# ebu/libear

Measured on AMD Instinct MI355X. Metric: Msamples/s, higher is better.
Workload: dtype f32 io / f16x2-split MFMA, f32 accumulate

## Files before the change

include/earhip.h:

```cpp
#ifndef EARHIP_H
#define EARHIP_H

#include <stddef.h>
#include <stdint.h>

#ifdef __cplusplus
extern "C" {
#endif

#define EARHIP_VERSION 100

#define EARHIP_OK 0
#define EARHIP_INVALID_ARGUMENT 1
#define EARHIP_INTERNAL_ERROR 2
#define EARHIP_DEVICE_ERROR 3
#define EARHIP_NOT_IMPLEMENTED 4
#define EARHIP_UNKNOWN_LAYOUT 5
#define EARHIP_ADM_ERROR 6

int earhip_version(void);
const char *earhip_last_error(void);
int earhip_device_count(int *count);

typedef struct earhip_ctx earhip_ctx;
// ... 231 lines not shown
int earhip_render_process_frames_pcm(earhip_render *r, size_t nblocks, const void *frames,
                                     earhip_pcm_format fmt, int frame_channels, int first_channel,
                                     void *out_frames, const earhip_pcm_out *out);
int earhip_render_process_frames_pcm_device(earhip_render *r, size_t nblocks, const void *frames_dev,
                                            earhip_pcm_format fmt, int frame_channels,
                                            int first_channel, void *out_dev, size_t out_frame_bytes,
                                            size_t out_first_byte, const earhip_pcm_out *out);
int earhip_render_output_levels(earhip_render *r, float *peak, uint64_t *clipped, int reset);
int earhip_render_enable_timing(earhip_render *r, int enable);
int earhip_render_get_timing(earhip_render *r, double out[6]);
int earhip_render_gain_kernel(const earhip_render *r, int *kind);
int earhip_render_hinge_standby(earhip_render *r, int *standby);
int earhip_render_hinge_robust(earhip_render *r, int *robust);
int earhip_render_wide_form(earhip_render *r, int *wide);
int earhip_render_last_plan(const earhip_render *r, int out[4]);
int earhip_render_last_list_layout(const earhip_render *r, int *paired);
int earhip_render_last_tail_blocks(const earhip_render *r, int *blocks);
int earhip_render_last_host_chunks(const earhip_render *r, int *chunks);
int earhip_render_scratch_bytes(const earhip_render *r, size_t *bytes);

typedef struct earhip_comm earhip_comm;
int earhip_comm_unique_id(void *id128);
int earhip_comm_create(earhip_ctx *ctx, int rank, int world, const void *id128, earhip_comm **out);
int earhip_comm_destroy(earhip_comm *comm);
int earhip_comm_channel_range(int n_out, int rank, int world, int *padded_rows, int *lo, int *hi);
int earhip_render_exchange_device(earhip_comm *comm, int slot, const float *partial_dev,
                                  float *owned_dev, size_t rows_per_rank, size_t row_stride);
int earhip_comm_gather_device(earhip_comm *comm, int slot, const float *owned_dev, float *full_dev,
                              size_t rows_per_rank, size_t row_stride, int root);
int earhip_comm_wait(earhip_comm *comm, int slot);
// ... 39 lines not shown
```

libear_amd/capi.py:

```python
import ctypes as C
import os

import numpy as np

from .build import lib_path

f32p = C.POINTER(C.c_float)
i64p = C.POINTER(C.c_int64)
pp_f32 = C.POINTER(f32p)

OK, INVALID_ARGUMENT, INTERNAL_ERROR, DEVICE_ERROR, NOT_IMPLEMENTED, UNKNOWN_LAYOUT, ADM_ERROR = 0, 1, 2, 3, 4, 5, 6


class EarHipError(Exception):
    def __init__(self, code, msg):
        super().__init__(msg)
        self.code = code


class InvalidArgument(EarHipError, ValueError):
    """maps to ear::invalid_argument"""


class InternalError(EarHipError, RuntimeError):
# ... 829 lines not shown
    def last_host_chunks(self):
        v = C.c_int(0)
        check(load().earhip_render_last_host_chunks(self.h, C.byref(v)))
        return v.value

    def last_list_layout(self):
        v = C.c_int(0)
        check(load().earhip_render_last_list_layout(self.h, C.byref(v)))
        return None if v.value < 0 else bool(v.value)

    def last_plan(self):
        out = (C.c_int * 4)()
        check(load().earhip_render_last_plan(self.h, out))
        return {"kernel": out[0], "tile": out[1], "ntiles": out[2], "gsplit": out[3]}

    def attach_loudness(self, meter):
        check(load().earhip_render_attach_loudness(self.h, meter.h if meter is not None else None))
        self._meter = meter

    def close(self):
        if self.h:
            load().earhip_render_destroy(self.h)
            self.h = C.c_void_p()



def _f64(a):
    return np.ascontiguousarray(a, dtype=np.float64)


# ... 106 lines not shown
```

libear_amd/csrc/api_core.hip:

```cpp
#include <cctype>
#include <cerrno>
#include <cmath>
#include <cstdlib>
#include <string>
#include <memory>
#include <mutex>

#include "common.h"
#include "curves.h"
#include "gain_kernels.h"
#include "gain_mfma.h"
#include "gain_h2.h"
#include "gain_h2_t1.h"
#include "gain_p2.h"
#include "gain_hg.h"
#include "gain_f32g.h"

namespace earhip {

static_assert(kSplitTile == 256, "MixLaunch::tile() and tiles_aligned(256, ...) assume the 4-wave tile");

static thread_local std::string g_last_error;
void set_last_error(const std::string &msg) { g_last_error = msg; }

// ... 140 lines not shown
    const dim3 bgrid((pnt + tpw - 1) / tpw);
    PairRec *stage = nullptr;
    if (ctx->has(OPT_BUILD_2K) ? ctx->get(OPT_BUILD_2K) != 0 : ml.paired) {
      stage = reinterpret_cast<PairRec *>(desc) + piece_units((size_t)M, (size_t)pnt, (size_t)pl.slots);
      hipLaunchKernelGGL(k_piece_classify, dim3((pnt + 63) / 64, (M + kClassifyObjects - 1) / kClassifyObjects), dim3(64 * kClassifyObjects), 0,
                         ctx->stream, ps, M, pnt, ptile, t_call, t_call + nsamples, pl.paired, stage, obj_lv, level_cur,
                         ml.hinge ? gate : nullptr);
    }
#define EARHIP_BUILD_CASE(T_)                                                                                          \
  if (tpw == T_)                                                                                                       \
    hipLaunchKernelGGL(k_piece_build<T_>, bgrid, dim3(kBuildThreads), 0, ctx->stream, ps, M, pnt, ptile, t_call, \
                       t_call + nsamples, pl, obj_lv, level_cur, ml.hinge ? gate : nullptr, ctx->obj_level_cap, wide_cur, stage);
    EARHIP_BUILD_CASE(1) EARHIP_BUILD_CASE(2) EARHIP_BUILD_CASE(4) EARHIP_BUILD_CASE(8)
#undef EARHIP_BUILD_CASE
  }
  if (!fused_prep && !one_pass) {
    const dim3 ogrid((M + 15) / 16);
    QuietMark qm;
    if (probe.obj_level) {
      qm.obj_level = probe.obj_level, qm.cap = ctx->obj_level_cap, qm.level = level_cur;
      qm.wide = ml.split ? wide_cur : nullptr;
    }
    if (ml.ntiles >= 2048)
      hipLaunchKernelGGL(k_seg_prep<4>, dim3((ml.ntiles + 63) / 64, ogrid.x), dim3(256), 0, ctx->stream, ps, M,
                         ml.ntiles, ml.tile(), t_call, t_call + nsamples, desc, qm, slow_cur);
    else
      hipLaunchKernelGGL(k_seg_prep<2>, dim3((ml.ntiles + 31) / 32, ogrid.x), dim3(256), 0, ctx->stream, ps, M,
                         ml.ntiles, ml.tile(), t_call, t_call + nsamples, desc, qm, slow_cur);
  }
  SlotLists sl;
  sl.slots = reinterpret_cast<Slot *>(desc + (size_t)M * ml.ntiles);
// ... 1 lines not shown
  sl.ovf = sl.count + (size_t)4 * ml.ntiles;
  sl.M = M;
  if (slots)
    hipLaunchKernelGGL(k_slot_list, dim3(ml.ntiles), dim3(256), 0, ctx->stream, ps, M, ml.tile(),
                       t_call, t_call + nsamples, fused_prep ? nullptr : desc, sl);
  if (ev) EARHIP_HIP(hipEventRecord(ev[1], ctx->stream));
  GainMixParams P;
  P.mode_word = gate;
  P.record = gate ? record : nullptr;
  P.sl = sl;
  P.in = in_dev;
  P.in_stride = in_stride;
  P.out = out_dev;
  P.out_stride = out_stride;
  P.part_stride = part_stride;
  P.desc = desc;
  P.ps = ps;
  P.t_call = t_call;
  P.nsamples = nsamples;
  P.ntiles = ml.ntiles;
  P.M = M;
  P.ncols = cs.ncols();
  P.ngroups = ml.mfma ? cp.mgroups : cp.ngroups;
  P.wsplit = ml.wsplit;
  P.tiles_per_wg = ml.mfma ? ml.tpw : 1;
  P.vec_ok = (in_stride % 4 == 0 && out_stride % 4 == 0 && part_stride % 4 == 0 &&
              ((uintptr_t)in_dev & 15) == 0 && ((uintptr_t)out_dev & 15) == 0)
                 ? 1
                 : 0;
  const dim3 grid(ml.mfma ? (ml.ntiles + ml.tpw - 1) / ml.tpw : ml.ntiles, ml.gsplit,
                  ml.mfma ? cp.mnz : cp.nz);
// ... 111 lines not shown
#undef EARHIP_MIX_CASE
  if (!launched) fail_internal("no gain_mix instantiation for this column plan");
  if (ev) EARHIP_HIP(hipEventRecord(ev[3], ctx->stream));
  EARHIP_HIP(hipGetLastError());
}

void reserve_call_words(earhip_ctx *ctx, int M, size_t max_samples) {
  if (!ctx->level.p) ctx->level.alloc_zero(4, ctx->stream);
  const size_t ntiles = (max_samples + 255) / 256;
  const bool grow_obj = ctx->obj_level_cap < M, grow_tiles = ctx->tile_slow_cap < ntiles;
  if (grow_obj || grow_tiles) EARHIP_HIP(hipStreamSynchronize(ctx->stream));
  if (grow_obj) {
    ctx->obj_level_cap = M + M / 2 + 64;
    ctx->obj_level.alloc_zero(2 * (size_t)ctx->obj_level_cap, ctx->stream);
  }
  if (grow_tiles) {
    ctx->tile_slow_cap = std::max<size_t>(ntiles + ntiles / 4, 1024);
    ctx->tile_slow.alloc_zero(2 * ctx->tile_slow_cap, ctx->stream);
    ctx->tile_slow_idx = 0;
  }
}

size_t hinge_build_allow_lds(const hipDeviceProp_t &prop) {
  const size_t want = 128 * 1024, dflt = 64 * 1024;
  const size_t device_max = std::max((size_t)prop.sharedMemPerBlock, (size_t)prop.maxSharedMemoryPerMultiProcessor);
  size_t ask = std::min(want, device_max > 4096 ? device_max - 4096 : dflt);
  if (ask <= dflt) return dflt;
  bool ok = true;
#define EARHIP_HBUILD_ATTR(T_, NW_)                                                                       \
  ok = ok && hipFuncSetAttribute(reinterpret_cast<const void *>(&k_hinge_build<T_, NW_>),                 \
// ... 58 lines not shown
    run_device(t_call, n, ctx->dev_in.p, stride, ctx->dev_out.p, stride);
    EARHIP_HIP(hipMemcpyAsync(ctx->pin_out.p, ctx->dev_out.p, sizeof(float) * stride * n_out,
                              hipMemcpyDeviceToHost, ctx->stream));
    EARHIP_HIP(hipStreamSynchronize(ctx->stream));
    for (int c = 0; c < n_out; c++)
      std::memcpy(out[c] + r0, ctx->pin_out.p + c * stride, sizeof(float) * n);
  }
};

}

using namespace earhip;

static const char *const kOptNames[OPT_COUNT] = {
    "SPL", "MFMA", "XSCALE", "WAVES", "TPW", "NRT", "H2_TILE", "H2_WGS", "H2_RUNS", "P2_TILE", "P2_PAIRS", "P2_WGS", "HINGE", "HG_TILE", "HBUILD_TPW",
    "BUILD_TPW", "K2_WG", "K2_OWN_BLOCK", "RUN", "GSPLIT", "PROBE_RUNS", "BLOCK_GROUPS", "DEBUG_TIMING", "TAILCUT", "HOST_CHUNK_MB", "HOST_THREADS", "HG_ROBUST", "BUILD_2K", "HOST_BIND", "HOST_NT", "HOST_FIRST", "H2_PAIR"};

static int parse_option_value(const std::string &key, const char *text) {
  char *end = nullptr;
  errno = 0;
  const long v = std::strtol(text, &end, 10);
  while (end && *end && std::isspace((unsigned char)*end)) end++;
  if (end == text || (end && *end) || errno == ERANGE || v < -(1L << 30) || v > (1L << 30))
    fail_invalid("option '" + key + "': '" + std::string(text) + "' is not an integer");
  return (int)v;
}

void earhip_ctx::apply_options() {
  spl = 4, use_mfma = 3, x_scale_log2 = 14, x_scale_auto = true, max_waves = 4, tiles_per_wg = 4, tiles_per_wg_forced = false, nrt = 8;
  if (has(OPT_SPL) && (get(OPT_SPL) == 2 || get(OPT_SPL) == 4)) spl = get(OPT_SPL);
  if (has(OPT_MFMA)) use_mfma = get(OPT_MFMA);
// ... 474 lines not shown
```

libear_amd/csrc/api_render.hip:

```cpp
#include <cmath>
#include <cstdlib>
#include <atomic>
#include <chrono>
#include <condition_variable>
#include <memory>
#include <mutex>
#include <thread>
#include <vector>


#include "common.h"
#include "curves.h"
#include "host_gather.h"
#include "pcm_kernels.h"
#include "pcm_out_kernels.h"
#include "fft_kernels.h"
#include "render_kernels.h"

using namespace earhip;

namespace earhip {
std::vector<cf> make_twiddles(int L) {
  std::vector<cf> tw(L);
  const double pi = 3.14159265358979323846264338327950288;
// ... 221 lines not shown
    }
    (void)hipStreamDestroy(in);
    (void)hipStreamDestroy(out);
  }
};

struct earhip_render {
  earhip_ctx *ctx = nullptr;
  int M = 0, N = 0, B = 0, K = 1, D = 0, T = 0;
  int Bk = 0, Lk = 0;
  int NP = 1;
  std::unique_ptr<CurveSet> curves;
  int64_t t = 0;
  int last_plan[3] = {0, 0, 0};
  int last_paired = -1;
  size_t last_scratch_bytes = 0;
  long scratch_regrows = 0;
  DevBuf<unsigned> rec;
  bool last_gated = false;
  bool last_device_form = false;
  bool last_hg_robust = false;
  int last_kind = -1;
  int run_len = 11;
  bool run_len_set = false;

  DevBuf<SegDesc> desc;
  DevBuf<float> bus;
  int max_gsplit = 1;
  DevBuf<cf> H, tw;
  DevBuf<float> tail[2], dly[2], hist[2];
// ... 266 lines not shown
        P.accumulate = part > 0 ? 1 : 0;
        if (wave_k2) {
          hipLaunchKernelGGL(k_decorrelate_wave, dim3((grid.x + kDecorWaves - 1) / kDecorWaves, grid.y), dim3(64 * kDecorWaves),
                             0, ctx->stream, P);
          EARHIP_HIP(hipGetLastError());
        } else {
          launch_decor(Lk, P, grid, ctx->stream, true);
        }
      }
      if (evp) EARHIP_HIP(hipEventRecord(evp[5], ctx->stream));
      cur ^= 1;
      fresh = false;
    }
    if (timed) pending.push_back(pd);
    last_gated = ctx->last_gate_idx >= 0;
    last_device_form = ctx->last_wide_idx >= 0;
    last_hg_robust = last_gated && ctx->last_hinge_robust;
    if (ctx->lazy_allocs != lazy_before) scratch_regrows++;
    t += nsamples;
  }
};

extern "C" {

int earhip_render_create(earhip_ctx *ctx, const earhip_render_config *cfg, earhip_render **out) {
  return guarded([&] {
    require(ctx != nullptr && cfg != nullptr && out != nullptr, "NULL argument");
    require(cfg->n_objects >= 1 && cfg->n_out >= 1, "n_objects and n_out must be >= 1");
    require(cfg->n_buses == 1 || cfg->n_buses == 2, "n_buses must be 1 or 2");
    FftShape shape;
// ... 706 lines not shown

int earhip_render_last_host_chunks(const earhip_render *r, int *chunks) {
  return guarded([&] {
    require(r != nullptr && chunks != nullptr, "NULL argument");
    *chunks = r->last_host_chunks;
  });
}

int earhip_render_last_list_layout(const earhip_render *r, int *paired) {
  return guarded([&] {
    require(r != nullptr && paired != nullptr, "NULL argument");
    *paired = r->last_paired;
  });
}

int earhip_render_last_plan(const earhip_render *r, int out[4]) {
  return guarded([&] {
    require(r != nullptr && out != nullptr, "NULL argument");
    out[0] = r->last_kind;
    for (int i = 0; i < 3; i++) out[1 + i] = r->last_plan[i];
  });
}

}
```

libear_amd/csrc/common.h:

```cpp
#pragma once

#include <hip/hip_runtime.h>

#include <cstdint>
#include <cstdio>
#include <string>
#include <vector>

#include "../../include/earhip.h"

namespace earhip {

struct Error {
  int code;
  std::string msg;
};

void set_last_error(const std::string &msg);

template <typename F>
int guarded(F &&f) {
  try {
    f();
    return EARHIP_OK;
// ... 79 lines not shown
};

}

struct earhip_vbs;
namespace earhip {
void vbs_orphan(earhip_vbs *v);
}

namespace earhip {
enum Opt {
  OPT_SPL, OPT_MFMA, OPT_XSCALE, OPT_WAVES, OPT_TPW, OPT_NRT,
  OPT_H2_TILE, OPT_H2_WGS, OPT_H2_RUNS, OPT_P2_TILE, OPT_P2_PAIRS, OPT_P2_WGS, OPT_HINGE, OPT_HG_TILE, OPT_HBUILD_TPW, OPT_BUILD_TPW,
  OPT_K2_WG, OPT_K2_OWN_BLOCK, OPT_RUN, OPT_GSPLIT,
  OPT_PROBE_RUNS, OPT_BLOCK_GROUPS, OPT_DEBUG_TIMING, OPT_TAILCUT, OPT_HOST_CHUNK_MB, OPT_HOST_THREADS, OPT_HG_ROBUST, OPT_BUILD_2K,
  OPT_HOST_BIND, OPT_HOST_NT, OPT_HOST_FIRST, OPT_H2_PAIR, OPT_COUNT
};
struct OptVal {
  bool set = false;
  int v = 0;
};
}

struct earhip_ctx {
  earhip::OptVal opt[earhip::OPT_COUNT];
  bool has(earhip::Opt o) const { return opt[o].set; }
  int get(earhip::Opt o, int dflt = 0) const { return opt[o].set ? opt[o].v : dflt; }
  void apply_options();
  int device = 0;
  hipStream_t stream = nullptr;
  bool own_stream = false;
  bool strict = false;
  int spl = 4;
  int use_mfma = 3;
  int x_scale_log2 = 14;
  bool x_scale_auto = true;
  earhip::DevBuf<unsigned> level;
  int level_idx = 0;
  int last_gate_idx = -1;
  bool last_hinge_robust = false;
  int last_wide_idx = -1;
  earhip::DevBuf<unsigned> tile_slow;
  size_t tile_slow_cap = 0;
  int tile_slow_idx = 0;
  earhip::DevBuf<unsigned> obj_level;
  int obj_level_cap = 0;
  long lazy_allocs = 0;
  unsigned *record_slot = nullptr;
  int max_waves = 4;
  int tiles_per_wg = 4;
  bool tiles_per_wg_forced = false;
  int nrt = 8;
  int num_cus = 256;
  size_t hinge_build_lds = 64 * 1024;
  struct HostRange {
    const char *base;
    size_t bytes;
    bool owned;
  };
  std::vector<HostRange> host_ranges;
  std::vector<earhip_vbs *> pinned_adapters;
// ... 24 lines not shown
```

libear_amd/csrc/curves.h:

```cpp
#pragma once

#include <chrono>
#include <cmath>
#include <cstdio>
#include <cstdlib>

#include <algorithm>
#include <cstring>
#include <vector>

#include "common.h"
#include "gain_kernels.h"
#include "gain_p2.h"
#include "gain_hg.h"
#include "gain_f32g.h"

namespace earhip {

struct ColumnPlan {
  int nout = 24;
  int ngroups = 1;
  int nz = 1;
  int nct = 1;
  int mgroups = 1;
  int mnz = 1;
  int row = 24;
  static ColumnPlan make(int ncols) {
    ColumnPlan p;
    int groups = (ncols + 23) / 24;
    const int per = (ncols + groups - 1) / groups;
// ... 25 lines not shown
  if (threadIdx.x == 0) dst.off[m] = off, dst.cnt[m] = n, dst.hdr[m] = src.hdr[m];
  for (int i = threadIdx.x; i < n; i += 256) {
    dst.time[off + i] = src.time[off + i];
    dst.flat[off + i] = src.flat[off + i];
    dst.rec[off + i] = src.rec[off + i];
  }
  const size_t g0 = (size_t)off * row, gn = (size_t)n * row;
  const float4 *sg = reinterpret_cast<const float4 *>(src.gain + g0);
  float4 *dg = reinterpret_cast<float4 *>(dst.gain + g0);
  for (size_t i = threadIdx.x; i < gn / 4; i += 256) dg[i] = sg[i];
}

class CurveSet {
 public:
  CurveSet(int M, int ncols, int nbus = 1, bool force_ramp = false)
      : M_(M), ncols_(ncols), nbus_(nbus), force_ramp_(force_ramp), plan_(ColumnPlan::make(ncols)), obj_(M) {
    for (int m = 0; m < M; m++) {
      obj_[m].t.assign(1, 0);
      obj_[m].g.assign(plan_.row, 0.0f);
      obj_[m].flat.assign(1, 0);
      obj_[m].dirty = true;
      dirty_list_.push_back(m);
    }
    cmax_.assign(plan_.row, 0.0f);
    obj_cmax_.assign((size_t)M * plan_.row, 0.0f);
    cm_scratch_.assign(plan_.row, 0.0f);
    shrunk_cols_.assign(plan_.row, 0);
    dirty_list_.reserve(M);
    for (auto &p : phases_) p.items.reserve(M);
  }
  ~CurveSet() {
// ... 135 lines not shown
      h_cnt_.p[m] = n;
      h_hdr_.p[m] = ObjHdr{o.off, n, o.t[0], o.t[n - 1], 0};
      std::memcpy(h_time_.p + o.off, o.t.data(), (size_t)n * sizeof(int64_t));
      std::memcpy(h_flat_.p + o.off, o.flat.data(), (size_t)n);
      std::memcpy(h_gain_.p + (size_t)o.off * row, o.g.data(), (size_t)n * row * sizeof(float));
      for (int k = 0; k < n; k++) {
        PointRec &r = h_rec_.p[o.off + k];
        r.time = o.t[k];
        const int64_t len = k ? o.t[k] - o.t[k - 1] : 0;
        r.scale = len > 0 ? 1.0f / (float)len : 0.0f;
        r.flat = o.flat[k];
      }
      float *cm = obj_cmax_.data() + (size_t)m * row;
      if (o.has_stats) cmax_shrunk = retire(o.st, cm) || cmax_shrunk;
      o.st = stats_of(o, cm);
      admit(o.st, cm);
      o.has_stats = true;
    }
    if (cmax_shrunk) {
      for (size_t c = 0; c < row; c++) {
        if (!shrunk_cols_[c]) continue;
        shrunk_cols_[c] = 0;
        float v = 0.0f;
        for (int m = 0; m < M_; m++) {
          const float a = obj_cmax_[(size_t)m * row + c];
          v = a <= v ? v : a;
        }
        cmax_[c] = v;
      }
    }
// ... 64 lines not shown

  int aligned_tile(int64_t t_call) const {
    const int grids[2] = {512, 256};
    for (int gi = 0; gi < 2; gi++) {
      const int64_t G = grids[gi];
      const int si = 1 - gi;
      int off_grid_limit = M_ / 64;
      if (ramp_share() < 0.5) {
        const double deltas = deltas_per_pair(si ? 512 : 256);
        off_grid_limit = (int)(M_ * std::min(1.0 / 64, deltas / 200.0));
      }
      if (tiles_aligned((int)G, t_call)) return (int)G;
      if (grid_off_[gi] <= off_grid_limit && (((t_call - grid_phase_[gi]) % G) + G) % G == 0) return (int)G;
    }
    return 0;
  }

  double deltas_per_pair(int tile) const {
    const int gi = tile >= 512 ? 1 : 0;
    return tot_.tiles[gi] > 0 ? tot_.incid[gi] / tot_.tiles[gi] * moving_share() : 0.0;
  }
  double moving_share() const { return M_ > 0 ? (double)tot_.moving / M_ : 0.0; }
  double point_density_all() const { return point_density() * moving_share(); }
  double ramp_share() const { return tot_.span > 0 ? tot_.ramp / tot_.span : 0.0; }
  double point_density() const { return tot_.span > 0 ? tot_.npts / tot_.span : 0.0; }
  double pair_waste(int tile) const {
    const int gi = tile >= 512 ? 1 : 0;
    return (tot_.incid[gi] - tot_.touched[gi]) / std::max(1.0, tot_.tiles[gi] + tot_.incid[gi]);
  }
  double hinge_exact_share(size_t in_stride, size_t nsamples) const {
// ... 171 lines not shown
        uint64_t b = g;
        while (a) {
          const uint64_t r = b % a;
          b = a;
          a = r;
        }
        g = b;
      };
      for (int m = 0; m < M_ && g != 1; m++) {
        const ObjStats &s = obj_[m].st;
        fold(s.gcd);
        fold((uint64_t)(s.first >= t_ref_ ? s.first - t_ref_ : t_ref_ - s.first));
      }
      grid_ = g;
      grid_stale_ = false;
    }
    for (int gi = 0; gi < 2; gi++) {
      int64_t best = 0;
      int best_n = 0;
      for (const auto &kv : phases_[gi].items)
        if (kv.second > best_n) best_n = kv.second, best = kv.first;
      grid_phase_[gi] = best;
      grid_off_[gi] = M_ - best_n;
    }
    float gmax = 0.0f;
    for (float v : cmax_) gmax = v <= gmax ? gmax : v;
    gain_max_ = gmax;
  }

  int M_, ncols_, nbus_;
  bool force_ramp_;
  ColumnPlan plan_;
  std::vector<Obj> obj_;
  std::vector<int> dirty_list_;
  bool uploaded_once_ = false;
  size_t arena_used_ = 2, arena_cap_ = 0, abandoned_ = 0;
  struct Totals {
    double span = 0, ramp = 0, npts = 0, bad = 0, points = 0;
    long moving = 0;
    double incid[2] = {0, 0}, touched[2] = {0, 0}, tiles[2] = {0, 0};
    long sum_r15[2] = {0, 0}, sum_r7[2] = {0, 0};
  } tot_;
  struct PhaseCounts {
    std::vector<std::pair<int64_t, int>> items;
    void add(int64_t phase, int d) {
      for (size_t i = 0; i < items.size(); i++)
        if (items[i].first == phase) {
          items[i].second += d;
          if (items[i].second <= 0) items[i] = items.back(), items.pop_back();
// ... 149 lines not shown
```

libear_amd/csrc/gain_h2.h:

```cpp
#pragma once

#include <hip/hip_runtime.h>

#include <type_traits>

#include "gain_kernels.h"
#include "gain_mfma.h"

namespace earhip {

typedef uint32_t u32x4 __attribute__((ext_vector_type(4)));
typedef float f32x2 __attribute__((ext_vector_type(2)));

constexpr int kSplitTile = 256;
constexpr int kSplitChunk = 32;

typedef _Float16 f16x8 __attribute__((ext_vector_type(8)));
typedef _Float16 f16x2_t __attribute__((ext_vector_type(2)));

__device__ __forceinline__ uint32_t pack_f16(float a, float b) {
  const f32x2 v = {a, b};
  return __builtin_bit_cast(uint32_t, __builtin_convertvector(v, f16x2_t));
}
__device__ __forceinline__ float f16_lo(uint32_t u) { return (float)__builtin_bit_cast(f16x2_t, u)[0]; }
// ... 220 lines not shown
      const int ts0 = st.tile * (TS * NW);
      const char *bp = reinterpret_cast<const char *>(P.in + (live ? (size_t)chunk_base(st.c) * P.in_stride + ts0 : 0));
      const size_t rstride = live ? P.in_stride * sizeof(float) : 0;
      const unsigned xo = live ? xrow + 4u * (unsigned)min(xsl, nvec - 4 - ts0) : 0u;
#pragma unroll
      for (int q = 0; q < 8; q++)
        if (q >= q0 && q < q0 + n)
          x[q] = __builtin_nontemporal_load(reinterpret_cast<const f32x4 *>(bp + (size_t)q * rstride + xo));
    };
    auto load_x = [&](const Stage &st, bool live, f32x4 (&x)[8]) { load_x_part(st, live, x, 0, 8); };
    typedef const SegDesc __attribute__((address_space(4))) *ConstDesc;
    struct ChunkDesc {
      SegDesc d[NQ];
    };
    auto load_desc = [&](const Stage &st) {
      ConstDesc dp = (ConstDesc)(P.desc + (size_t)st.tile * P.M + chunk_base(st.c) + w * NQ);
      ChunkDesc D;
#pragma unroll
      for (int q = 0; q < NQ; q++) {
        D.d[q].row = dp[q].row;
        D.d[q].d0 = dp[q].d0;
        D.d[q].scale = dp[q].scale;
        D.d[q].info = dp[q].info;
      }
      return D;
    };
    struct ChunkCoef {
      float p0[NQ], scale[NQ];
    };
    auto load_gains = [&](const ChunkDesc &R, int cc, ChunkCoef &D, float (&S)[NQ], float (&E)[NQ]) {
      const int m0 = chunk_base(cc) + w * NQ;
#pragma unroll
      for (int q = 0; q < NQ; q++) {
        const SegDesc d = R.d[q];
        const bool valid = m0 + q >= m_lo + cc * CH && !(d.info & (kSegMulti | kSegQuiet));
        const unsigned rs = (unsigned)(valid ? d.row : zero_row);
        const unsigned re = (valid && (d.info & kSegRamp)) ? (unsigned)d.row + 1u : rs;
        D.p0[q] = d.scale != 0.0f ? (float)(d.d0 + (TS * NW) / 2) * d.scale : 0.0f;
        D.scale[q] = d.scale;
        const float *rps = gain + (size_t)rs * rowlen, *rpe = gain + (size_t)re * rowlen;
        S[q] = rps[bcol_e];
        E[q] = rpe[bcol_e];
      }
    };
    auto store_b = [&](const ChunkCoef &D, const float (&S)[NQ], const float (&E)[NQ], int buf, int part) {
      uint32_t h[NQ / 2], l[NQ / 2], hs[NQ / 2];
#pragma unroll
      for (int i = 0; i < NQ / 2; i++) {
        float v[2];
// ... 22 lines not shown
      }
    };

    f32x4 X0[8], X1[8];
    ChunkDesc L;
    Stage sa, sb, sc;
    sa.tile = tile_at(vb_c);
    sa.c = 0;
    sb = next_stage(sa);
    sc = next_stage(sb);
    int ka = 0;
    {
      float S[NQ], E[NQ];
      ChunkCoef D;
      L = load_desc(sa);
      load_gains(L, 0, D, S, E);
      load_x(sa, true, X0);
      load_x(sb, left > 1, X1);
      store_b(D, S, E, 0, 0);
      store_b(D, S, E, 0, 1);
      L = load_desc(sb);
    }
    auto chunk = [&](int buf, f32x4 (&xc)[8]) __attribute__((always_inline)) {
      __syncthreads();
      float S[NQ], E[NQ];
      ChunkCoef D;
      load_gains(L, sb.c, D, S, E);
      L = load_desc(sc);
      __builtin_amdgcn_sched_barrier(0);

      u32x4 ah[NRT], al[NRT];
#pragma unroll
      for (int qp = 0; qp < 4; qp++)
#pragma unroll
        for (int rp = 0; rp < NRT; rp += 2) {
          const f32x2 s0 = f32x2{xc[2 * qp][rp], xc[2 * qp][rp + 1]} * x_scale;
          const f32x2 s1 = f32x2{xc[2 * qp + 1][rp], xc[2 * qp + 1][rp + 1]} * x_scale;
          const uint32_t H0 = pack_f16(s0[0], s1[0]), H1 = pack_f16(s0[1], s1[1]);
          constexpr float LOW = WIDE ? kLowPieceScale : 1.0f;
          const f32x2 r0 = f32x2{sub_f16_lo(s0[0], H0), sub_f16_lo(s0[1], H1)} * LOW;
          const f32x2 r1 = f32x2{sub_f16_hi(s1[0], H0), sub_f16_hi(s1[1], H1)} * LOW;
          ah[rp][qp] = H0;
// ... 54 lines not shown
            __builtin_amdgcn_sched_group_barrier(0x002, 2, 0);
            __builtin_amdgcn_sched_group_barrier(0x020, 1, 0);
          }
        } else {
          __builtin_amdgcn_sched_group_barrier(0x008, 12, 0);
        }
      }
    };
    auto tile_end = [&](int t) __attribute__((always_inline)) {
      {
        typedef const unsigned __attribute__((address_space(4))) *ConstWord;
        const bool any_slow = !slow_cur || ((ConstWord)slow_cur)[t] != 0u;
        if (slow_next && blockIdx.y == 0 && blockIdx.z == 0 && threadIdx.x == 0) slow_next[t] = 0u;
        for (int b0 = 0; any_slow && b0 < nobj; b0 += 64) {
          const int ol = opaque_lane();
          const SegDesc db = (P.desc + (size_t)t * P.M)[min(m_lo + b0 + ol, m_hi - 1)];
          unsigned long long multi = __ballot((db.info & (kSegMulti | kSegQuiet)) && b0 + ol < nobj);
          while (multi) {
            const int j = __builtin_ctzll(multi);
            multi &= multi - 1;
            single_object(t, m_lo + b0 + j, x_scale, true, seg_k(__shfl(db.info, j)));
          }
        }
        bool bad = false;
#pragma unroll
        for (int r = 0; r < NRT; r++)
#pragma unroll
          for (int c = 0; c < NCT; c++)
#pragma unroll
            for (int e = 0; e < 4; e++) bad |= !(__builtin_fabsf(tot0[r][c][e]) < INFINITY) || !(__builtin_fabsf(tot1[r][c][e]) < INFINITY);
        if (__ballot(bad)) {
// ... 42 lines not shown
```

libear_amd/csrc/gain_h2_t1.h:

```cpp
#pragma once

#include "gain_h2.h"

namespace earhip {

template <int NCT, int NW, bool WIDE>
__global__ void __launch_bounds__(64 * NW, 2)
k_gain_mix_h2_t1(GainMixParams P, int zero_row, float x_scale, const float *__restrict__ gcol, const unsigned *level_cur,
              unsigned *level_next, const unsigned *slow_cur, unsigned *slow_next, const unsigned *wide_cur, unsigned *wide_next) {
  if (wide_cur && ((*wide_cur & 1u) != 0u) != WIDE) return;
  constexpr int NRT = 4, TS = 16 * NRT, CH = kSplitChunk;
  constexpr int NQ = CH / NW;
  constexpr int NFRAG = 2 * NCT * 3;
  __shared__ u32x4 bfrag[2][NFRAG + 6][64];
  constexpr int OP = TS + 4;
  __shared__ __attribute__((aligned(16))) float otile[NW][16 * OP];
  __shared__ float inv_gcol[16 * NCT];
  if (threadIdx.x < 16 * NCT) inv_gcol[threadIdx.x] = 1.0f / gcol[blockIdx.z * 16 * NCT + threadIdx.x];
  __syncthreads();
  const int lane = threadIdx.x & 63;
  const int w = __builtin_amdgcn_readfirstlane(threadIdx.x >> 6);
  const int li = lane & 15, kg = lane >> 4;
  const int wgtile = xcd_tile(blockIdx.x, gridDim.x);
  if (blockIdx.x == 0 && blockIdx.y == 0 && blockIdx.z == 0 && threadIdx.x == 0) {
// ... 7 lines not shown
      x_scale = __uint_as_float((unsigned)(127 + 7 - E) << 23);
    }
    if (blockIdx.x == 0 && blockIdx.y == 0 && blockIdx.z == 0 && threadIdx.x == 0) *level_next = 0;
  }
  const bool any_slow = !slow_cur || slow_cur[wgtile] != 0u;
  if (slow_next && blockIdx.y == 0 && blockIdx.z == 0 && threadIdx.x == 0) slow_next[wgtile] = 0u;
  const int nparts = gridDim.y;
  const int part = blockIdx.y;
  const int m_lo = (int)(((int64_t)P.M * part) / nparts);
  const int m_hi = (int)(((int64_t)P.M * (part + 1)) / nparts);
  const int col0 = blockIdx.z * 16 * NCT;
  const int tile_s0 = wgtile * (TS * NW) + w * TS;
  const int tile_len = max(0, min(TS, P.nsamples - tile_s0));
  const int64_t tile_t0 = P.t_call + tile_s0;
  const int64_t tile_t1 = tile_t0 + tile_len;
  const SegDesc *__restrict__ dtile = P.desc + (size_t)wgtile * P.M;
  const float *__restrict__ gain = P.ps.gain;
  const unsigned rowlen = (unsigned)P.ps.row;

  f32x4 tot0[NRT][NCT], tot1[NRT][NCT];
  auto clear_totals = [&]() {
#pragma unroll
    for (int r = 0; r < NRT; r++)
#pragma unroll
      for (int c = 0; c < NCT; c++) tot0[r][c] = tot1[r][c] = f32x4{0.0f, 0.0f, 0.0f, 0.0f};
  };
  clear_totals();

  auto single_object = [&](int m, float sx, bool sg, int khint = -1) {
    if (tile_len <= 0) return;
    float gsc[NCT];
// ... 82 lines not shown
        D.d[q].row = dp[q].row;
        D.d[q].d0 = dp[q].d0;
        D.d[q].scale = dp[q].scale;
        D.d[q].info = dp[q].info;
      }
      return D;
    };
    struct ChunkCoef {
      float p0[NQ], scale[NQ];
    };
    auto load_gains = [&](const ChunkDesc &R, int c, ChunkCoef &D, float (&S)[NQ], float (&E)[NQ]) {
      const int cc = min(c, nch - 1);
      const int m0 = chunk_base(cc) + w * NQ;
#pragma unroll
      for (int q = 0; q < NQ; q++) {
        const SegDesc d = R.d[q];
        const bool valid = m0 + q >= m_lo + cc * CH && !(d.info & (kSegMulti | kSegQuiet));
        const unsigned rs = (unsigned)(valid ? d.row : zero_row);
        const unsigned re = (valid && (d.info & kSegRamp)) ? (unsigned)d.row + 1u : rs;
        D.p0[q] = d.scale != 0.0f ? (float)(d.d0 + (TS * NW) / 2) * d.scale : 0.0f;
        D.scale[q] = d.scale;
        const float *rps = gain + (size_t)rs * rowlen, *rpe = gain + (size_t)re * rowlen;
        S[q] = rps[bcol_e];
        E[q] = rpe[bcol_e];
      }
    };
    auto store_b = [&](const ChunkCoef &D, const float (&S)[NQ], const float (&E)[NQ], int buf, int part) {
      uint32_t h[NQ / 2], l[NQ / 2], hs[NQ / 2];
#pragma unroll
      for (int i = 0; i < NQ / 2; i++) {
        float v[2];
// ... 112 lines not shown
            __builtin_amdgcn_sched_group_barrier(0x002, 2, 0);
            __builtin_amdgcn_sched_group_barrier(0x020, 1, 0);
          }
        } else {
          __builtin_amdgcn_sched_group_barrier(0x008, 12, 0);
        }
      }
    };
#pragma unroll 1
    for (int c = 0; c < nch; c += 2) {
      chunk(c, 0, X0);
      if (c + 1 < nch) chunk(c + 1, 1, X1);
    }

    for (int b0 = 0; any_slow && b0 < nobj; b0 += 64) {
      const SegDesc db = dtile[min(m_lo + b0 + lane, m_hi - 1)];
      unsigned long long multi = __ballot((db.info & (kSegMulti | kSegQuiet)) && b0 + lane < nobj);
      while (multi) {
        const int j = __builtin_ctzll(multi);
        multi &= multi - 1;
        single_object(m_lo + b0 + j, x_scale, true, seg_k(__shfl(db.info, j)));
      }
    }
    bool bad = false;
#pragma unroll
    for (int r = 0; r < NRT; r++)
#pragma unroll
      for (int c = 0; c < NCT; c++)
#pragma unroll
        for (int e = 0; e < 4; e++) bad |= !(__builtin_fabsf(tot0[r][c][e]) < INFINITY) || !(__builtin_fabsf(tot1[r][c][e]) < INFINITY);
    if (__ballot(bad)) {
// ... 61 lines not shown
```

libear_amd/csrc/gain_kernels.h:

```cpp
#pragma once

#include <hip/hip_runtime.h>

#include <cstdint>

#include "search.h"

namespace earhip {

struct PointRec {
  int64_t time;
  float scale;
  uint32_t flat;
};
static_assert(sizeof(PointRec) == 16, "PointRec is loaded as one dwordx4");

struct ObjHdr {
  int32_t off, cnt;
  int64_t first, last;
  int64_t reserved;
};
static_assert(sizeof(ObjHdr) == 32, "an object's header is two dwordx4 loads");
struct PointStore {
  const ObjHdr *hdr;
// ... 212 lines not shown
        while (k < n && ps.rec[base + k].time <= t0) k++;
      }
      SegDesc d = describe_segment_rec(ps, base, n, k, t0, t_end);
      if (quiet) d.info |= kSegQuiet;
      sh[ti * kPrepRun + j][oi] = d;
      if (tile_slow && (quiet || (d.info & kSegMulti))) atomicOr(&tile_slow[tile], 1u);
    }
  }
  __syncthreads();
#pragma unroll
  for (int j = 0; j < kPrepRun; j++) {
    const int to = (threadIdx.x >> 4) + 16 * j, oo = threadIdx.x & 15;
    const int tile_o = blockIdx.x * 16 * kPrepRun + to, m_o = blockIdx.y * 16 + oo;
    if (tile_o < ntiles && m_o < M) desc[(size_t)tile_o * M + m_o] = sh[to][oo];
  }
}

struct Slot {
  uint32_t mr;
  int32_t row;
  float alpha, beta;
};
static_assert(sizeof(Slot) == 16, "Slot is loaded as one dwordx4");
constexpr int kMaxSlotObjects = 1 << 16;
constexpr int kPlainSlots = 2;
constexpr int kMaskedSlots = 6;
constexpr int kTileSlots = kPlainSlots + kMaskedSlots;
struct SlotLists {
  Slot *slots;
  int *count;
// ... 131 lines not shown
  }
  if (tid == 0) {
    sl.count[tile * 4 + 0] = base_p;
    sl.count[tile * 4 + 1] = written_m;
    sl.count[tile * 4 + 2] = base_o;
  }
}

struct GainMixParams {
  const float *in;
  size_t in_stride;
  float *out;
  size_t out_stride;
  size_t part_stride;
  const SegDesc *desc;
  PointStore ps;
  int64_t t_call;
  int nsamples;
  int ntiles;
  int M;
  int ncols;
  int ngroups;
  int wsplit;
  int tiles_per_wg;
  int vec_ok;
  SlotLists sl;
  int tile_runs = 0;
  const unsigned *mode_word = nullptr;
  unsigned *record = nullptr;
};
constexpr unsigned kModeRecorded = 4u;
__device__ __forceinline__ void record_mode(const GainMixParams &P, bool device_form) {
  if (P.record) *P.record = (P.mode_word ? *P.mode_word : 0u) | (device_form ? 0u : 1u) | kModeRecorded;
}

template <int NOUT, int SPL, bool STRICT, bool PARTIAL>
__device__ __forceinline__ void accumulate_piece(float (&acc)[NOUT][SPL], const float (&xs)[SPL], const bool (&on)[SPL],
                                                 const SegDesc d, const float *__restrict__ rows,
                                                 int rowlen, int lane, int col0, int bus_cols) {
  const bool ramp = d.info & kSegRamp;
  const float *__restrict__ S = rows;
  const float *__restrict__ E = rows + (ramp ? rowlen : 0);
  float p[SPL], q[SPL];
#pragma unroll
  for (int i = 0; i < SPL; i++) {
    p[i] = (float)(d.d0 + lane * SPL + i) * d.scale;
    q[i] = 1.0f - p[i];
  }
// ... 175 lines not shown
```

Baseline: 1.103 million.

## Replace per-tile segment descriptors with per-object records stepped analytically for regular calls

New measurement: 1.054 million. -4.5%, worse.

```diff
diff --git a/include/earhip.h b/include/earhip.h
--- a/include/earhip.h
+++ b/include/earhip.h
@@ -269,6 +269,7 @@
 int earhip_render_hinge_robust(earhip_render *r, int *robust);
 int earhip_render_wide_form(earhip_render *r, int *wide);
 int earhip_render_last_plan(const earhip_render *r, int out[4]);
+int earhip_render_last_descriptors(const earhip_render *r, int out[8]);
 int earhip_render_last_list_layout(const earhip_render *r, int *paired);
 int earhip_render_last_tail_blocks(const earhip_render *r, int *blocks);
 int earhip_render_last_host_chunks(const earhip_render *r, int *chunks);
diff --git a/libear_amd/capi.py b/libear_amd/capi.py
--- a/libear_amd/capi.py
+++ b/libear_amd/capi.py
@@ -867,6 +867,12 @@
         check(load().earhip_render_last_plan(self.h, out))
         return {"kernel": out[0], "tile": out[1], "ntiles": out[2], "gsplit": out[3]}
 
+    def last_descriptors(self):
+        out = (C.c_int * 8)()
+        check(load().earhip_render_last_descriptors(self.h, out))
+        span = lambda o: None if out[o] < 0 else {"regular": bool(out[o]), "log2p": out[o + 1], "phase": out[o + 2], "why": out[o + 3]}
+        return {"main": span(0), "tail": span(4)}
+
     def attach_loudness(self, meter):
         check(load().earhip_render_attach_loudness(self.h, meter.h if meter is not None else None))
         self._meter = meter
diff --git a/libear_amd/csrc/api_core.hip b/libear_amd/csrc/api_core.hip
--- a/libear_amd/csrc/api_core.hip
+++ b/libear_amd/csrc/api_core.hip
@@ -178,7 +178,26 @@
     EARHIP_BUILD_CASE(1) EARHIP_BUILD_CASE(2) EARHIP_BUILD_CASE(4) EARHIP_BUILD_CASE(8)
 #undef EARHIP_BUILD_CASE
   }
-  if (!fused_prep && !one_pass) {
+  RegularCall rc;
+  if (ml.split && ml.gsplit == 1 && !strict && !fused_prep && !one_pass && ctx->get(OPT_DESC_GENERAL, 0) == 0)
+    rc = cs.regular_call(t_call, nsamples, ml.tile());
+  ctx->last_desc[0] = rc.regular ? 1 : 0, ctx->last_desc[1] = rc.regular ? rc.log2p : 0, ctx->last_desc[2] = rc.regular ? rc.phase : 0;
+  ctx->last_desc[3] = rc.why;
+  SegDesc *obj_rec = nullptr;
+  if (rc.regular) {
+    if (ctx->obj_rec_cap < M) {
+      EARHIP_HIP(hipStreamSynchronize(ctx->stream));
+      ctx->obj_rec_cap = M + M / 2 + 64;
+      ctx->obj_rec.alloc((size_t)ctx->obj_rec_cap);
+      ctx->lazy_allocs++;
+    }
+    obj_rec = reinterpret_cast<SegDesc *>(ctx->obj_rec.p);
+    QuietMark qm;
+    if (probe.obj_level) qm.obj_level = probe.obj_level, qm.cap = ctx->obj_level_cap, qm.level = level_cur, qm.wide = wide_cur;
+    hipLaunchKernelGGL(k_obj_prep, dim3((M + 255) / 256), dim3(256), 0, ctx->stream, ps, M, ml.ntiles, ml.tile(), t_call,
+                       t_call + nsamples, obj_rec, qm, slow_cur);
+  }
+  if (!fused_prep && !one_pass && !rc.regular) {
     const dim3 ogrid((M + 15) / 16);
     QuietMark qm;
     if (probe.obj_level) {
@@ -210,7 +229,9 @@
   P.out = out_dev;
   P.out_stride = out_stride;
   P.part_stride = part_stride;
-  P.desc = desc;
+  P.desc = obj_rec ? obj_rec : desc;
+  P.desc_stride = obj_rec ? 0 : M;
+  P.rec_walk = obj_rec ? (rc.phase | (rc.log2p << 24)) : 0;
   P.ps = ps;
   P.t_call = t_call;
   P.nsamples = nsamples;
@@ -352,6 +373,11 @@
     ctx->obj_level_cap = M + M / 2 + 64;
     ctx->obj_level.alloc_zero(2 * (size_t)ctx->obj_level_cap, ctx->stream);
   }
+  if (ctx->obj_rec_cap < M) {
+    if (!(grow_obj || grow_tiles)) EARHIP_HIP(hipStreamSynchronize(ctx->stream));
+    ctx->obj_rec_cap = M + M / 2 + 64;
+    ctx->obj_rec.alloc((size_t)ctx->obj_rec_cap);
+  }
   if (grow_tiles) {
     ctx->tile_slow_cap = std::max<size_t>(ntiles + ntiles / 4, 1024);
     ctx->tile_slow.alloc_zero(2 * ctx->tile_slow_cap, ctx->stream);
@@ -440,7 +466,7 @@
 
 static const char *const kOptNames[OPT_COUNT] = {
     "SPL", "MFMA", "XSCALE", "WAVES", "TPW", "NRT", "H2_TILE", "H2_WGS", "H2_RUNS", "P2_TILE", "P2_PAIRS", "P2_WGS", "HINGE", "HG_TILE", "HBUILD_TPW",
-    "BUILD_TPW", "K2_WG", "K2_OWN_BLOCK", "RUN", "GSPLIT", "PROBE_RUNS", "BLOCK_GROUPS", "DEBUG_TIMING", "TAILCUT", "HOST_CHUNK_MB", "HOST_THREADS", "HG_ROBUST", "BUILD_2K", "HOST_BIND", "HOST_NT", "HOST_FIRST", "H2_PAIR"};
+    "BUILD_TPW", "K2_WG", "K2_OWN_BLOCK", "RUN", "GSPLIT", "PROBE_RUNS", "BLOCK_GROUPS", "DEBUG_TIMING", "TAILCUT", "HOST_CHUNK_MB", "HOST_THREADS", "HG_ROBUST", "BUILD_2K", "HOST_BIND", "HOST_NT", "HOST_FIRST", "H2_PAIR", "DESC_GENERAL"};
 
 static int parse_option_value(const std::string &key, const char *text) {
   char *end = nullptr;
diff --git a/libear_amd/csrc/api_render.hip b/libear_amd/csrc/api_render.hip
--- a/libear_amd/csrc/api_render.hip
+++ b/libear_amd/csrc/api_render.hip
@@ -259,6 +259,7 @@
   int64_t t = 0;
   int last_plan[3] = {0, 0, 0};
   int last_paired = -1;
+  int last_desc[2][4] = {{0, 0, 0, 0}, {-1, 0, 0, 0}};
   size_t last_scratch_bytes = 0;
   long scratch_regrows = 0;
   DevBuf<unsigned> rec;
@@ -555,6 +556,8 @@
     }
     if (timed) pending.push_back(pd);
     last_gated = ctx->last_gate_idx >= 0;
+    for (int i = 0; i < 4; i++) last_desc[continues ? 1 : 0][i] = ctx->last_desc[i];
+    if (!continues) last_desc[1][0] = -1, last_desc[1][1] = last_desc[1][2] = last_desc[1][3] = 0;
     last_device_form = ctx->last_wide_idx >= 0;
     last_hg_robust = last_gated && ctx->last_hinge_robust;
     if (ctx->lazy_allocs != lazy_before) scratch_regrows++;
@@ -1291,6 +1294,14 @@
   });
 }
 
+int earhip_render_last_descriptors(const earhip_render *r, int out[8]) {
+  return guarded([&] {
+    require(r != nullptr && out != nullptr, "NULL argument");
+    for (int s = 0; s < 2; s++)
+      for (int i = 0; i < 4; i++) out[4 * s + i] = r->last_desc[s][i];
+  });
+}
+
 int earhip_render_last_plan(const earhip_render *r, int out[4]) {
   return guarded([&] {
     require(r != nullptr && out != nullptr, "NULL argument");
diff --git a/libear_amd/csrc/common.h b/libear_amd/csrc/common.h
--- a/libear_amd/csrc/common.h
+++ b/libear_amd/csrc/common.h
@@ -117,7 +117,7 @@
   OPT_H2_TILE, OPT_H2_WGS, OPT_H2_RUNS, OPT_P2_TILE, OPT_P2_PAIRS, OPT_P2_WGS, OPT_HINGE, OPT_HG_TILE, OPT_HBUILD_TPW, OPT_BUILD_TPW,
   OPT_K2_WG, OPT_K2_OWN_BLOCK, OPT_RUN, OPT_GSPLIT,
   OPT_PROBE_RUNS, OPT_BLOCK_GROUPS, OPT_DEBUG_TIMING, OPT_TAILCUT, OPT_HOST_CHUNK_MB, OPT_HOST_THREADS, OPT_HG_ROBUST, OPT_BUILD_2K,
-  OPT_HOST_BIND, OPT_HOST_NT, OPT_HOST_FIRST, OPT_H2_PAIR, OPT_COUNT
+  OPT_HOST_BIND, OPT_HOST_NT, OPT_HOST_FIRST, OPT_H2_PAIR, OPT_DESC_GENERAL, OPT_COUNT
 };
 struct OptVal {
   bool set = false;
@@ -148,6 +148,9 @@
   int tile_slow_idx = 0;
   earhip::DevBuf<unsigned> obj_level;
   int obj_level_cap = 0;
+  earhip::DevBuf<uint4> obj_rec;
+  int obj_rec_cap = 0;
+  int last_desc[4] = {0, 0, 0, 0};
   long lazy_allocs = 0;
   unsigned *record_slot = nullptr;
   int max_waves = 4;
diff --git a/libear_amd/csrc/curves.h b/libear_amd/csrc/curves.h
--- a/libear_amd/csrc/curves.h
+++ b/libear_amd/csrc/curves.h
@@ -14,6 +14,7 @@
 #include "gain_p2.h"
 #include "gain_hg.h"
 #include "gain_f32g.h"
+#include "regular_call.h"
 
 namespace earhip {
 
@@ -69,7 +70,7 @@
 class CurveSet {
  public:
   CurveSet(int M, int ncols, int nbus = 1, bool force_ramp = false)
-      : M_(M), ncols_(ncols), nbus_(nbus), force_ramp_(force_ramp), plan_(ColumnPlan::make(ncols)), obj_(M) {
+      : M_(M), ncols_(ncols), nbus_(nbus), force_ramp_(force_ramp), plan_(ColumnPlan::make(ncols)), obj_(M), shapes_(M) {
     for (int m = 0; m < M; m++) {
       obj_[m].t.assign(1, 0);
       obj_[m].g.assign(plan_.row, 0.0f);
@@ -235,6 +236,7 @@
       float *cm = obj_cmax_.data() + (size_t)m * row;
       if (o.has_stats) cmax_shrunk = retire(o.st, cm) || cmax_shrunk;
       o.st = stats_of(o, cm);
+      shapes_[m] = obj_shape(o.t.data(), o.flat.data(), n, (1 << nbus_) - 1);
       admit(o.st, cm);
       o.has_stats = true;
     }
@@ -329,6 +331,11 @@
       if (grid_off_[gi] <= off_grid_limit && (((t_call - grid_phase_[gi]) % G) + G) % G == 0) return (int)G;
     }
     return 0;
+  }
+
+  RegularCall regular_call(int64_t t_call, int nsamples, int tile) const {
+    if (force_ramp_ || !dirty_list_.empty()) return RegularCall();
+    return classify_regular_call(shapes_.data(), M_, facts_, t_call, nsamples, tile);
   }
 
   double deltas_per_pair(int tile) const {
@@ -530,6 +537,7 @@
       }
       grid_ = g;
       grid_stale_ = false;
+      facts_ = fold_shapes(shapes_.data(), M_);
     }
     for (int gi = 0; gi < 2; gi++) {
       int64_t best = 0;
@@ -549,6 +557,8 @@
   ColumnPlan plan_;
   std::vector<Obj> obj_;
   std::vector<int> dirty_list_;
+  std::vector<ObjShape> shapes_;
+  RegularSetFacts facts_;
   bool uploaded_once_ = false;
   size_t arena_used_ = 2, arena_cap_ = 0, abandoned_ = 0;
   struct Totals {
diff --git a/libear_amd/csrc/gain_h2.h b/libear_amd/csrc/gain_h2.h
--- a/libear_amd/csrc/gain_h2.h
+++ b/libear_amd/csrc/gain_h2.h
@@ -258,7 +258,7 @@
       SegDesc d[NQ];
     };
     auto load_desc = [&](const Stage &st) {
-      ConstDesc dp = (ConstDesc)(P.desc + (size_t)st.tile * P.M + chunk_base(st.c) + w * NQ);
+      ConstDesc dp = (ConstDesc)(desc_row(P, st.tile) + chunk_base(st.c) + w * NQ);
       ChunkDesc D;
 #pragma unroll
       for (int q = 0; q < NQ; q++) {
@@ -272,11 +272,11 @@
     struct ChunkCoef {
       float p0[NQ], scale[NQ];
     };
-    auto load_gains = [&](const ChunkDesc &R, int cc, ChunkCoef &D, float (&S)[NQ], float (&E)[NQ]) {
+    auto load_gains = [&](const ChunkDesc &R, int t, int cc, ChunkCoef &D, float (&S)[NQ], float (&E)[NQ]) {
       const int m0 = chunk_base(cc) + w * NQ;
 #pragma unroll
       for (int q = 0; q < NQ; q++) {
-        const SegDesc d = R.d[q];
+        const SegDesc d = desc_step(P, R.d[q], t, TS * NW);
         const bool valid = m0 + q >= m_lo + cc * CH && !(d.info & (kSegMulti | kSegQuiet));
         const unsigned rs = (unsigned)(valid ? d.row : zero_row);
         const unsigned re = (valid && (d.info & kSegRamp)) ? (unsigned)d.row + 1u : rs;
@@ -329,7 +329,7 @@
       float S[NQ], E[NQ];
       ChunkCoef D;
       L = load_desc(sa);
-      load_gains(L, 0, D, S, E);
+      load_gains(L, sa.tile, 0, D, S, E);
       load_x(sa, true, X0);
       load_x(sb, left > 1, X1);
       store_b(D, S, E, 0, 0);
@@ -340,7 +340,7 @@
       __syncthreads();
       float S[NQ], E[NQ];
       ChunkCoef D;
-      load_gains(L, sb.c, D, S, E);
+      load_gains(L, sb.tile, sb.c, D, S, E);
       L = load_desc(sc);
       __builtin_amdgcn_sched_barrier(0);
 
@@ -425,7 +425,7 @@
         if (slow_next && blockIdx.y == 0 && blockIdx.z == 0 && threadIdx.x == 0) slow_next[t] = 0u;
         for (int b0 = 0; any_slow && b0 < nobj; b0 += 64) {
           const int ol = opaque_lane();
-          const SegDesc db = (P.desc + (size_t)t * P.M)[min(m_lo + b0 + ol, m_hi - 1)];
+          const SegDesc db = desc_step(P, desc_row(P, t)[min(m_lo + b0 + ol, m_hi - 1)], t, TS * NW);
           unsigned long long multi = __ballot((db.info & (kSegMulti | kSegQuiet)) && b0 + ol < nobj);
           while (multi) {
             const int j = __builtin_ctzll(multi);
diff --git a/libear_amd/csrc/gain_h2_t1.h b/libear_amd/csrc/gain_h2_t1.h
--- a/libear_amd/csrc/gain_h2_t1.h
+++ b/libear_amd/csrc/gain_h2_t1.h
@@ -45,7 +45,7 @@
   const int tile_len = max(0, min(TS, P.nsamples - tile_s0));
   const int64_t tile_t0 = P.t_call + tile_s0;
   const int64_t tile_t1 = tile_t0 + tile_len;
-  const SegDesc *__restrict__ dtile = P.desc + (size_t)wgtile * P.M;
+  const SegDesc *__restrict__ dtile = desc_row(P, wgtile);
   const float *__restrict__ gain = P.ps.gain;
   const unsigned rowlen = (unsigned)P.ps.row;
 
@@ -158,7 +158,7 @@
       const int m0 = chunk_base(cc) + w * NQ;
 #pragma unroll
       for (int q = 0; q < NQ; q++) {
-        const SegDesc d = R.d[q];
+        const SegDesc d = desc_step(P, R.d[q], wgtile, TS * NW);
         const bool valid = m0 + q >= m_lo + cc * CH && !(d.info & (kSegMulti | kSegQuiet));
         const unsigned rs = (unsigned)(valid ? d.row : zero_row);
         const unsigned re = (valid && (d.info & kSegRamp)) ? (unsigned)d.row + 1u : rs;
@@ -301,7 +301,7 @@
     }
 
     for (int b0 = 0; any_slow && b0 < nobj; b0 += 64) {
-      const SegDesc db = dtile[min(m_lo + b0 + lane, m_hi - 1)];
+      const SegDesc db = desc_step(P, dtile[min(m_lo + b0 + lane, m_hi - 1)], wgtile, TS * NW);
       unsigned long long multi = __ballot((db.info & (kSegMulti | kSegQuiet)) && b0 + lane < nobj);
       while (multi) {
         const int j = __builtin_ctzll(multi);
diff --git a/libear_amd/csrc/gain_kernels.h b/libear_amd/csrc/gain_kernels.h
--- a/libear_amd/csrc/gain_kernels.h
+++ b/libear_amd/csrc/gain_kernels.h
@@ -250,6 +250,46 @@
     const int tile_o = blockIdx.x * 16 * kPrepRun + to, m_o = blockIdx.y * 16 + oo;
     if (tile_o < ntiles && m_o < M) desc[(size_t)tile_o * M + m_o] = sh[to][oo];
   }
+}
+
+constexpr int kSegStep = kSegMulti;
+static __global__ void __launch_bounds__(256)
+k_obj_prep(PointStore ps, int M, int ntiles, int tile_samples, int64_t t_call, int64_t t_call_end, SegDesc *rec, QuietMark qm,
+           unsigned *tile_slow) {
+  const int m = blockIdx.x * 256 + threadIdx.x;
+  bool quiet = false, wide = false;
+  if (qm.obj_level && m < M) {
+    const unsigned call = *qm.level, lv = qm.obj_level[m], lo = qm.obj_level[qm.cap + m];
+    quiet = level_is_quiet(lv, call);
+    wide = qm.wide && lo != 0u && call != 0u && (int)(lo >> 23) < (int)(call >> 23) - kPlainBinades;
+  }
+  if (m < M) {
+    const ObjHdr hd = ps.hdr[m];
+    const int base = hd.off, n = hd.cnt;
+    const int k = upper_bound_rec_window(ps.rec + base, n, hd.first, hd.last, t_call);
+    int64_t t_end = t_call + tile_samples;
+    if (t_end > t_call_end) t_end = t_call_end;
+    SegDesc d = describe_segment_rec(ps, base, n, k, t_call, t_end);
+    d.info &= ~kSegMulti;
+    if (k < n && ps.rec[base + k].time < t_call_end) d.info |= kSegStep;
+    if (quiet) d.info |= kSegQuiet;
+    rec[m] = d;
+  }
+  const int any_quiet = __syncthreads_or(quiet ? 1 : 0);
+  if (tile_slow && any_quiet)
+    for (int j = threadIdx.x; j < ntiles; j += 256) tile_slow[j] = 1u;
+  if (__syncthreads_or(wide ? 1 : 0) && threadIdx.x == 0) atomicOr(qm.wide, 1u);
+}
+__host__ __device__ __forceinline__ SegDesc step_record(SegDesc r, int i, int tile, int log2p, int phase) {
+  const bool step = (r.info & kSegStep) != 0, ramp = (r.info & kSegRamp) != 0;
+  const int ip = i + phase;
+  const int s = step ? ip >> log2p : 0;
+  SegDesc d;
+  d.row = r.row + s;
+  d.d0 = ramp ? (step ? (ip & ((1 << log2p) - 1)) * tile : r.d0 + i * tile) : 0;
+  d.scale = r.scale;
+  d.info = (r.info & ~kSegStep) + (s << 13);
+  return d;
 }
 
 struct Slot {
@@ -411,6 +451,8 @@
   size_t out_stride;
   size_t part_stride;
   const SegDesc *desc;
+  int desc_stride = 0;
+  int rec_walk = 0;
   PointStore ps;
   int64_t t_call;
   int nsamples;
@@ -429,6 +471,13 @@
 constexpr unsigned kModeRecorded = 4u;
 __device__ __forceinline__ void record_mode(const GainMixParams &P, bool device_form) {
   if (P.record) *P.record = (P.mode_word ? *P.mode_word : 0u) | (device_form ? 0u : 1u) | kModeRecorded;
+}
+
+__device__ __forceinline__ const SegDesc *desc_row(const GainMixParams &P, int t) {
+  return P.desc + (size_t)t * (size_t)P.desc_stride;
+}
+__device__ __forceinline__ SegDesc desc_step(const GainMixParams &P, SegDesc d, int t, int tile) {
+  return P.desc_stride == 0 ? step_record(d, t, tile, P.rec_walk >> 24, P.rec_walk & 0xffffff) : d;
 }
 
 template <int NOUT, int SPL, bool STRICT, bool PARTIAL>
diff --git a/libear_amd/csrc/regular_call.h b/libear_amd/csrc/regular_call.h
--- /dev/null
+++ b/libear_amd/csrc/regular_call.h
@@ -0,0 +1,140 @@
+#pragma once
+
+#include <algorithm>
+#include <cstdint>
+
+namespace earhip {
+
+struct ObjShape {
+  const int64_t *t = nullptr;
+  int32_t npoints = 0;
+  int32_t uflat = -1;
+  int64_t first = 0, last = 0;
+  int64_t ulen = 0;
+};
+
+inline ObjShape obj_shape(const int64_t *t, const uint8_t *flat, int n, int allflat) {
+  ObjShape s;
+  s.t = t;
+  s.npoints = n;
+  s.first = t[0];
+  s.last = t[n - 1];
+  if (n < 2) return s;
+  s.ulen = t[1] - t[0];
+  s.uflat = flat[1] & allflat;
+  for (int k = 2; k < n; k++) {
+    if (t[k] - t[k - 1] != s.ulen) s.ulen = 0;
+    if ((flat[k] & allflat) != s.uflat) s.uflat = -1;
+  }
+  if (s.ulen <= 0) s.ulen = 0;
+  return s;
+}
+
+enum RegularWhy {
+  kRegularYes = 0,
+  kRegularOffGrid = 1,
+  kRegularMixedPeriods = 2,
+  kRegularEndsInside = 3,
+  kRegularFlatVaries = 4,
+  kRegularIrregular = 5,
+  kRegularNotAsked = 6
+};
+struct RegularCall {
+  bool regular = false;
+  int log2p = 0;
+  int phase = 0;
+  int why = kRegularNotAsked;
+};
+
+struct RegularSetFacts {
+  int n_single = 0;
+  int n_uniform = 0;
+  int n_other = 0;
+  int64_t ulen = 0;
+  int64_t uphase = 0;
+  int64_t max_first = INT64_MIN, min_last = INT64_MAX;
+};
+inline int64_t floor_mod(int64_t a, int64_t m) { return ((a % m) + m) % m; }
+inline RegularSetFacts fold_shapes(const ObjShape *s, int M) {
+  RegularSetFacts F;
+  for (int m = 0; m < M; m++) {
+    const ObjShape &o = s[m];
+    if (o.npoints < 2) {
+      F.n_single++;
+    } else if (o.ulen > 0 && o.uflat >= 0) {
+      if (F.n_uniform == 0) F.ulen = o.ulen, F.uphase = floor_mod(o.first, o.ulen);
+      else if (F.ulen != o.ulen) F.ulen = -1;
+      else if (F.uphase != floor_mod(o.first, o.ulen)) F.uphase = -1;
+      F.n_uniform++;
+      F.max_first = std::max(F.max_first, o.first);
+      F.min_last = std::min(F.min_last, o.last);
+    } else {
+      F.n_other++;
+    }
+  }
+  return F;
+}
+
+namespace regular_detail {
+inline int fit_period(int64_t ulen, int64_t off, int tile, int &log2p, int &phase) {
+  if (off % tile != 0) return kRegularOffGrid;
+  if (ulen % tile != 0) return kRegularOffGrid;
+  const int64_t P = ulen / tile;
+  if (P > (1 << 20) || (P & (P - 1)) != 0) return kRegularMixedPeriods;
+  log2p = 0;
+  while (((int64_t)1 << log2p) < P) log2p++;
+  phase = (int)(off / tile);
+  return kRegularYes;
+}
+}
+
+inline RegularCall classify_regular_call(const ObjShape *shapes, int M, const RegularSetFacts &F, int64_t t_call,
+                                         int nsamples, int tile) {
+  RegularCall R;
+  R.why = kRegularYes;
+  const int64_t t0 = t_call, t1 = t_call + nsamples;
+  bool have_period = false;
+  auto periodic = [&](int64_t ulen, int64_t off) {
+    int l2 = 0, ph = 0;
+    const int why = regular_detail::fit_period(ulen, off, tile, l2, ph);
+    if (why != kRegularYes) return why;
+    if (have_period && (l2 != R.log2p || ph != R.phase)) return (int)kRegularMixedPeriods;
+    have_period = true, R.log2p = l2, R.phase = ph;
+    return (int)kRegularYes;
+  };
+  if (nsamples <= 0 || tile <= 0) {
+    R.why = kRegularNotAsked;
+    return R;
+  }
+  if (F.n_other == 0 && (F.n_uniform == 0 || (F.ulen > 0 && F.uphase >= 0 && F.max_first <= t0 && F.min_last >= t1))) {
+    if (F.n_uniform > 0) {
+      const int64_t off = floor_mod(t0 - F.uphase, F.ulen);
+      if (off + nsamples > F.ulen) R.why = periodic(F.ulen, off);
+    }
+    R.regular = R.why == kRegularYes;
+    return R;
+  }
+  for (int m = 0; m < M && R.why == kRegularYes; m++) {
+    const ObjShape &o = shapes[m];
+    if (o.npoints < 2 || o.first >= t1 || o.last <= t0) continue;
+    if (o.ulen > 0 && o.first <= t0 && o.last >= t1) {
+      const int64_t off = (t0 - o.first) % o.ulen;
+      if (off + nsamples <= o.ulen) continue;
+      R.why = o.uflat < 0 ? (int)kRegularFlatVaries : periodic(o.ulen, off);
+      continue;
+    }
+    const int64_t *e = std::upper_bound(o.t, o.t + o.npoints, t0);
+    if (e == o.t + o.npoints || *e >= t1) continue;
+    if (o.first > t0 || o.last < t1) R.why = kRegularEndsInside;
+    else R.why = kRegularIrregular;
+    for (const int64_t *p = e; p != o.t + o.npoints && *p < t1; p++)
+      if ((*p - t0) % tile != 0) {
+        R.why = kRegularOffGrid;
+        break;
+      }
+  }
+  R.regular = R.why == kRegularYes;
+  return R;
+}
+
+}
```
